# pabloruizponce/MixerMDM

Hardware: AMD Instinct MI355X
Metric: generated motions/sec (1000-step DDPM schedule sampled with DDIM eta=0, T=300, 2-person) (higher is better)
Workload: dtype f32; 1 GPU; BASELINE configs[2]: 2-person MixerMDM (in2IN individual + in2IN interaction + Mixer mode 4, align, CFG 3.5), T=300, ddim1000 (eta=0), batch 16 per GPU, fp32, random-init weights; batch_per_gpu=16, frames=300, sampler=ddim1000, sampler_steps=1000, hipgraph=True, parallelism=batch-sharded x1, no in-loop collective

## Files before the change

### include/mmdm.h

```cpp
#ifndef MMDM_H
#define MMDM_H

#include <stddef.h>
#include <stdint.h>

#ifdef __cplusplus
extern "C" {
#endif
#pragma GCC visibility push(default)

typedef enum {
    MMDM_OK = 0,
    MMDM_ERR_ARG = 1,
    MMDM_ERR_STATE = 2,
    MMDM_ERR_HIP = 3,
    MMDM_ERR_UNSUPPORTED = 4
} mmdm_status;

const char* mmdm_last_error(void);
const char* mmdm_version(void);
const char* mmdm_last_gemm_kernel(void);


enum {
// ... 205 lines not shown
    int noise_steps;
    const float* noise;
    const unsigned long long* item_seed;
    const int* item_noise_row;
    const float* x_start;
    const float* init_image;
    int init_zeros;
    float init_coef[2];
    int skip_timesteps;
} mmdm_begin_ragged_options;
int mmdm_begin_ragged_opts(mmdm_handle h, const float* cond, const float* x_T, int B, const int* lens_host, const mmdm_begin_ragged_options* opts, void* stream);
int mmdm_call_rows(mmdm_handle h, int* rows, int* real_rows, int* ragged);

int mmdm_set_history(mmdm_handle h, float* influence_i1, float* influence_i2, float* out1, float* out2, float* out_influenced, int every);

int mmdm_run(mmdm_handle h, int nsteps, int use_graph, void* stream);
int mmdm_graph_stats(mmdm_handle h, int64_t* captures, int64_t* replays, int* cached);
int mmdm_graph_parked(void);

int mmdm_seek(mmdm_handle h, int step_index, void* stream);

int mmdm_get_state(mmdm_handle h, float** x, float** x2, float** pred_xstart, float** pred_xstart2, float** model_out);

int mmdm_copy_result(mmdm_handle h, float* dst, void* stream);

int mmdm_module_forward(mmdm_handle h, int which, const float* x, const float* x2, const float* cond, int t,
                        float* out, int n, int T, void* stream);

int mmdm_profile_enable(mmdm_handle h, int on);
int mmdm_profile_read(mmdm_handle h, int which, double* total_ms, int64_t* launches, double* flops, double* algorithmic_bytes);

int mmdm_diag_set(const char* key, long long value);

#pragma GCC visibility pop
#ifdef __cplusplus
}
#endif
#endif
```

### mixermdm_amd/_lib.py

```python
import ctypes as C
import os

_HERE = os.path.dirname(os.path.abspath(__file__))
_LIB = None


class MMDMError(RuntimeError):

    def __init__(self, msg, status=0):
        super().__init__(msg)
        self.status = int(status)


def lib_path():
    return os.environ.get("MMDM_LIB") or os.path.join(_HERE, "libmmdm_hip.so")


def lib_override():
    return bool(os.environ.get("MMDM_LIB"))


class Config(C.Structure):
    _fields_ = [(n, C.c_int) for n in ("d_latent", "d_ff", "d_layers", "d_heads", "m_latent", "m_ff", "m_layers", "m_heads",
                                        "nfeats", "text_dim", "mixing_mode", "align", "xstart_align", "model2_kind", "use_force")] + \
# ... 71 lines not shown
    "mmdm_set_weight": (_I, [_VP, C.c_char_p, _VP, C.c_int64, C.c_int64, _VP]),
    "mmdm_set_norm_stats": (_I, [_VP, _VP]),
    "mmdm_set_schedule": (_I, [_VP, _VP, _VP, _I, _VP]),
    "mmdm_prepare": (_I, [_VP]),
    "mmdm_begin": (_I, [_VP, _VP, _VP, _I, _I, _VP]),
    "mmdm_set_eta": (_I, [_VP, _VP, _I]),
    "mmdm_begin_opts": (_I, [_VP, _VP, _VP, _I, _I, C.POINTER(BeginOptions), _VP]),
    "mmdm_randn_f32": (_I, [C.c_ulonglong, _I, _I, _I, _VP, _VP]),
    "mmdm_begin_ragged": (_I, [_VP, _VP, _VP, _I, _VP, _VP]),
    "mmdm_begin_ragged_opts": (_I, [_VP, _VP, _VP, _I, _VP, C.POINTER(BeginRaggedOptions), _VP]),
    "mmdm_call_rows": (_I, [_VP, C.POINTER(_I), C.POINTER(_I), C.POINTER(_I)]),
    "mmdm_attention_ragged_f32": (_I, [_VP, _I, _VP, _I, _VP, _I, _VP, _I, _I, _VP, _VP, _I, _I, _I, _I, _I, _VP]),
    "mmdm_attention_ragged_opts_f32": (_I, [_VP, _I, _VP, _I, _VP, _I, _VP, _I, _I, _I, _VP, _VP, _I, _I, _I, _I, _I, _VP]),
    "mmdm_attention_split_ragged": (_I, [_VP, _I, C.c_int64, _VP, _I, C.c_int64, _VP, _I, C.c_int64, _VP, _I, _I, _I, _I, _VP, _VP, _I, _I, _I, _I, _I, _VP]),
    "mmdm_layernorm_split": (_I, [_VP, _VP, _VP, _VP, _VP, C.c_int64, _I, _I, C.c_float, _I, _VP]),
    "mmdm_rowop_adaln": (_I, [_VP, _VP, _I, _I, _VP, _I, _VP, _I, _I, _I, _VP, _I, _I, _VP]),
    "mmdm_rowop_cond_silu": (_I, [_VP, _VP, _VP, _VP, _I, C.c_int64, _I, _I, _I, _VP]),
    "mmdm_rowop_mean_time": (_I, [_VP, _VP, _I, _I, _VP, _VP, _I, _I, _VP]),
    "mmdm_rowop_mdm_pack": (_I, [_VP, _VP, _I, _VP, _VP, _VP, _VP, _VP, C.c_int64, _I, _I, _I, _I, _VP]),
    "mmdm_rowop_mdm_unpack": (_I, [_VP, _VP, _I, _I, _I, _I, _VP]),
    "mmdm_rowop_mdm_pack_rag": (_I, [_VP, _VP, _I, _VP, _VP, _VP, _VP, _VP, C.c_int64, _I, _I, _I, _I] + [_I, _VP, _VP, _VP, _VP] * 2 + [_I, _VP]),
    "mmdm_rowop_mdm_unpack_rag": (_I, [_VP, _VP, _I, _I, _I] + [_I, _VP, _VP, _VP, _VP] * 2 + [_I, _VP]),
    "mmdm_set_history":(_I, [_VP, _VP, _VP, _VP, _VP, _VP, _I]),
    "mmdm_run": (_I, [_VP, _I, _I, _VP]),
    "mmdm_seek": (_I, [_VP, _I, _VP]),
    "mmdm_graph_stats": (_I, [_VP, C.POINTER(C.c_int64), C.POINTER(C.c_int64), C.POINTER(_I)]),
    "mmdm_graph_parked": (_I, []),
    "mmdm_last_gemm_kernel": (C.c_char_p, []),
    "mmdm_get_state": (_I, [_VP] + [C.POINTER(_VP)] * 5),
    "mmdm_copy_result": (_I, [_VP, _VP, _VP]),
    "mmdm_module_forward": (_I, [_VP, _I, _VP, _VP, _VP, _I, _VP, _I, _I, _VP]),
    "mmdm_profile_enable": (_I, [_VP, _I]),
    "mmdm_diag_set": (_I, [C.c_char_p, C.c_longlong]),
    "mmdm_profile_read": (_I, [_VP, _I, C.POINTER(C.c_double), C.POINTER(C.c_int64), C.POINTER(C.c_double), C.POINTER(C.c_double)]),
}


def load_library():
    global _LIB
    if _LIB is not None:
        return _LIB
    import torch
    path = lib_path()
    if not os.path.exists(path):
        raise MMDMError(f"{path} not found: build it with `python -m mixermdm_amd.build` (hipcc, gfx950). "
                        "There is no CPU fallback for the denoising path.")
    lib = C.CDLL(path)
    for name, (res, args) in SYMBOLS.items():
        fn = getattr(lib, name)
        fn.restype = res
        fn.argtypes = args
    _LIB = lib
    return lib


def diag(key, value):
    check(load_library().mmdm_diag_set(key.encode(), int(value)))


def check(rc, handle=None):
    if rc == 0:
        return
    lib = load_library()
    msg = (lib.mmdm_handle_error(handle) if handle else None) or lib.mmdm_last_error() or b""
    msg = msg.decode(errors="replace")
    if "Mixing mode not recognized" in msg or "Mode not recognized" in msg:
# ... 3 lines not shown
```

### mixermdm_amd/csrc/gemm_f32.hip

```cpp
#include <hip/hip_runtime.h>
#include <stdlib.h>
#include <string.h>
#include <type_traits>
#include "kernels.h"

namespace {

typedef float f32x16 __attribute__((ext_vector_type(16)));
typedef float f32x4 __attribute__((ext_vector_type(4)));
typedef unsigned u32x4 __attribute__((ext_vector_type(4)));

struct GemmArgs {
    const float* A; const float* W; const float* bias; float* C; const float* extra;
    int lda, ldw, ldc, ld_extra;
    int M, N, K, Kw, epilogue, period;
    int mt, nt;
    int ablate;
    unsigned long long* stamps;
};

template <int VEC, bool FULL>
__device__ __forceinline__ f32x4 load4(const float* __restrict__ base, int ld, int row, int nrows, int k, int K) {
    if (FULL) return *reinterpret_cast<const f32x4*>(base + (size_t)row * ld + k);
    f32x4 v = {0.f, 0.f, 0.f, 0.f};
// ... 145 lines not shown
                else if (p.epilogue == MMDM_EPI_BIAS_QUICKGELU) v = quick_gelu(v);
                else if (p.epilogue == MMDM_EPI_BIAS_SIGMOID) v = sigmoidf(v);
                p.C[(size_t)row * p.ldc + col] = v;
            }
        }
    }
}

template <int TM_, int TN_, int BK_ = 16, int NBUF_ = 2>
struct GCfg {
    static constexpr int WGM = TM_ / 10, WGN = TN_ / 10, TM = TM_ % 10, TN = TN_ % 10;
    static constexpr int NWAVES = WGM * WGN, THREADS = 64 * NWAVES;
    static constexpr int BM = 32 * TM * WGM, BN = 32 * TN * WGN, BK = BK_;
    static constexpr int A_FLOATS = BM * BK, B_FLOATS = BN * BK;
    static constexpr int NBUF = NBUF_;
    static constexpr int SMEM_BYTES = NBUF * (A_FLOATS + B_FLOATS) * 4;
    static constexpr int CPR = BK / 4;
    static constexpr int RPP = 64 / CPR;
    static constexpr int NA = BM / RPP, NB = BN / RPP;
    static constexpr int NI = (NA + NB) / NWAVES;
    static_assert((NA + NB) % NWAVES == 0, "pieces must divide evenly over the waves (counted vmcnt)");
    static constexpr int G = BK / 8;
};

typedef __attribute__((address_space(1))) const void* gptr_t;
typedef __attribute__((address_space(3))) void* lptr_t;

template <int CPR> __device__ __forceinline__ int swz_of(int r) { return CPR == 4 ? ((r >> 2) & 3) : ((r >> 1) & 7); }

template <int N> __device__ __forceinline__ void wait_vm() { asm volatile("s_waitcnt vmcnt(%0)" ::"n"(N) : "memory"); }

#if defined(__HIP_DEVICE_COMPILE__)
template <int TM_, int TN_, int BK_, int NBUF_, bool VEPI, int PIPE_, bool DIAG_>
__device__ __forceinline__ void gemm_tile(const GemmArgs& pp, float* smem, int swz, int bid) {
    using C_ = GCfg<TM_, TN_, BK_, NBUF_>;
    const GemmArgs& p = pp;
    unsigned long long* const p_stamps = DIAG_ ? pp.stamps : nullptr;
    const int p_ablate = DIAG_ ? pp.ablate : 0;
    constexpr int BM = C_::BM, BN = C_::BN, BK = C_::BK, TM = C_::TM, TN = C_::TN, CPR = C_::CPR, RPP = C_::RPP, NBUF = C_::NBUF;
    float* As = smem;
    float* Bs = smem + NBUF * C_::A_FLOATS;

    const int m0 = (swz / p.nt) * BM;
    const int n0 = (swz % p.nt) * BN;

    const int tid = threadIdx.x;
    const int lane = tid & 63;
    const int wave = __builtin_amdgcn_readfirstlane(tid >> 6);
    const int wm = wave / C_::WGN, wn = wave % C_::WGN;
    const int l31 = lane & 31, lh = lane >> 5;
    if (p_stamps && tid == 0) {
        p_stamps[8 * (size_t)bid + 0] = __builtin_amdgcn_s_memrealtime();
        p_stamps[8 * (size_t)bid + 3] = (unsigned long long)__builtin_amdgcn_s_getreg((4) | (0 << 6) | (31 << 11)) |
                                        ((unsigned long long)__builtin_amdgcn_s_getreg((20) | (0 << 6) | (3 << 11)) << 32);
    }

    constexpr int UA = C_::NA / C_::NWAVES;
    static_assert(C_::NA % C_::NWAVES == 0, "A pieces must divide evenly over the waves (compile-time operand of a piece)");
    int voff[C_::NI];
    int dst[C_::NI];
#pragma unroll
    for (int u = 0; u < C_::NI; ++u) {
        const int pq = wave + C_::NWAVES * u;
        const int prow = lane / CPR, pc = lane % CPR;
        const bool isa = u < UA;
        const int trow = (isa ? RPP * pq : RPP * (pq - C_::NA)) + prow;
        const int gch = pc ^ swz_of<CPR>(trow);
        if (isa) {
            const int rel = min(trow, p.M - 1 - m0);
            voff[u] = (rel * p.lda + 4 * gch) * 4;
            dst[u] = RPP * pq * BK;
        } else {
            const int rel = min(trow, p.N - 1 - n0);
            voff[u] = (rel * p.ldw + 4 * gch) * 4;
            dst[u] = NBUF * C_::A_FLOATS + RPP * (pq - C_::NA) * BK;
        }
    }
    const __amdgpu_buffer_rsrc_t rsA = __builtin_amdgcn_make_buffer_rsrc(const_cast<float*>(p.A + (size_t)m0 * p.lda), 0, 0xffffffff, 0x00020000);
    const __amdgpu_buffer_rsrc_t rsW = __builtin_amdgcn_make_buffer_rsrc(const_cast<float*>(p.W + (size_t)n0 * p.ldw), 0, 0xffffffff, 0x00020000);
    int koff = 0;
    auto stage_part = [&](int buf, auto u0c, auto u1c) {
        constexpr int u0 = decltype(u0c)::value, u1 = decltype(u1c)::value;
#pragma unroll
        for (int u = u0; u < u1; ++u) {
            const int boff = u < UA ? buf * C_::A_FLOATS : buf * C_::B_FLOATS;
            __builtin_amdgcn_raw_ptr_buffer_load_lds(u < UA ? rsA : rsW, (lptr_t)(smem + dst[u] + boff), 16, voff[u], koff, 0, 0);
        }
        if constexpr (u1 == C_::NI) koff += BK * 4;
    };
    auto stage = [&](int buf) { stage_part(buf, std::integral_constant<int, 0>{}, std::integral_constant<int, C_::NI>{}); };

    const int nkt = p.K / BK;
    constexpr bool LATE_R = PIPE_ != 0 && VEPI;
    f32x16 acc[TM][TN];
    if (VEPI) {
#pragma unroll
        for (int i = 0; i < TM; ++i) {
            const int row = m0 + wm * (32 * TM) + i * 32 + l31;
            const bool rok = row < p.M;
            const int er = p.epilogue == MMDM_EPI_BIAS_PE ? row % p.period : row;
            const bool ext = !LATE_R && (p.epilogue == MMDM_EPI_BIAS_RESID || p.epilogue == MMDM_EPI_BIAS_PE) && rok;
#pragma unroll
            for (int j = 0; j < TN; ++j)
#pragma unroll
                for (int qd = 0; qd < 4; ++qd) {
                    const int col = n0 + wn * (32 * TN) + j * 32 + 8 * qd + 4 * lh;
                    f32x4 v = {0.f, 0.f, 0.f, 0.f};
                    if (col < p.N) {
                        if (p.bias) v = *reinterpret_cast<const f32x4*>(p.bias + col);
                        if (ext) v += *reinterpret_cast<const f32x4*>(p.extra + (size_t)er * p.ld_extra + col);
                    }
#pragma unroll
                    for (int c = 0; c < 4; ++c) acc[i][j][4 * qd + c] = v[c];
                }
        }
    } else {
#pragma unroll
    for (int i = 0; i < TM; ++i)
#pragma unroll
        for (int j = 0; j < TN; ++j) {
            const int col = n0 + wn * (32 * TN) + j * 32 + l31;
            const bool cok = col < p.N;
            const float bv = (p.bias && cok) ? p.bias[col] : 0.f;
#pragma unroll
            for (int e = 0; e < 16; ++e) {
                float v = bv;
                if (p.epilogue == MMDM_EPI_BIAS_RESID || p.epilogue == MMDM_EPI_BIAS_PE) {
                    const int row = m0 + wm * (32 * TM) + i * 32 + (e & 3) + 8 * (e >> 2) + 4 * lh;
                    if (cok && row < p.M) {
                        const int er = p.epilogue == MMDM_EPI_BIAS_PE ? row % p.period : row;
                        v += p.extra[(size_t)er * p.ld_extra + col];
                    }
                }
                acc[i][j][e] = v;
            }
        }
    }

    if constexpr (PIPE_ != 0) {
#pragma unroll
        for (int t = 0; t < NBUF - 1; ++t) stage(t);
        wait_vm<(NBUF - 2) * C_::NI>();
    } else {
        asm volatile("s_waitcnt vmcnt(0)" ::: "memory");
    }
    if (p_stamps && tid == 0) {
        p_stamps[8 * (size_t)bid + 1] = __builtin_amdgcn_s_memrealtime();
        p_stamps[8 * (size_t)gridDim.x + 2 * bid] = __builtin_readcyclecounter();
    }
    const int sw = swz_of<CPR>(l31);
    const int a_row = (wm * (32 * TM) + l31) * BK;
    const int b_row = (wn * (32 * TN) + l31) * BK;

    f32x4 rv[LATE_R ? TM : 1][LATE_R ? TN : 1][4];
    if constexpr (PIPE_ != 0) {
        static_assert((C_::G == 2 || C_::G == 4) && NBUF >= 3 && NBUF <= 6, "pipelined loop: K step 16 or 32 (two / four k-groups), 3 to 6 stages");
        static_assert((C_::NI + 1) / 2 <= 4 * TM * TN - 1, "LDS-DMA pieces of a tile must fit behind the MFMAs of two k-groups");
        constexpr int NI = C_::NI;
        f32x4 a0[TM], b0[TN], a1[TM], b1[TN];
        auto rd = [&](int buf, int g, f32x4 (&af)[TM], f32x4 (&bf)[TN]) {
            const int cg = 4 * ((2 * g + lh) ^ sw);
            const float* Ac = As + buf * C_::A_FLOATS + a_row + cg;
            const float* Bc = Bs + buf * C_::B_FLOATS + b_row + cg;
// ... 49 lines not shown
            } else {
                if constexpr (g < G - 1) rd(cur, g + 1, a0, b0);
                else if (more) rd(nxt, 0, a0, b0);
                if constexpr (STG && g == 1 && PIPE_ != 2) stage_part(stg, std::integral_constant<int, D0>{}, std::integral_constant<int, NI>{});
                mm(a1, b1);
            }
            __builtin_amdgcn_sched_group_barrier(0x008, 1, g);
            __builtin_amdgcn_sched_group_barrier(0x100, TM + TN, g);
#pragma unroll
            for (int u = 0; u < dma_here; ++u) {
                __builtin_amdgcn_sched_group_barrier(0x008, 1, g);
                __builtin_amdgcn_sched_group_barrier(0x010, 1, g);
            }
            __builtin_amdgcn_sched_group_barrier(0x008, NMM - 1 - dma_here, g);
            __builtin_amdgcn_sched_barrier(0);
        };
        auto step = [&](auto do_stage, int left, bool more) {
            group(std::integral_constant<int, 0>{}, do_stage, left, more);
            group(std::integral_constant<int, 1>{}, do_stage, left, more);
            if constexpr (G >= 4) {
                group(std::integral_constant<int, 2>{}, do_stage, left, more);
                group(std::integral_constant<int, 3>{}, do_stage, left, more);
            }
            cur = nxt; nxt = nxt + 1 == NBUF ? 0 : nxt + 1;
        };
        for (int kt = 0; kt < n_main; ++kt) {
            step(std::true_type{}, 0, true);
            stg = stg + 1 == NBUF ? 0 : stg + 1;
        }
        if constexpr (LATE_R) {
#pragma unroll
            for (int i = 0; i < TM; ++i) {
                const int row = m0 + wm * (32 * TM) + i * 32 + l31;
                const int er = p.epilogue == MMDM_EPI_BIAS_PE ? row % p.period : row;
#pragma unroll
                for (int j = 0; j < TN; ++j)
#pragma unroll
                    for (int qd = 0; qd < 4; ++qd) {
                        const int col = n0 + wn * (32 * TN) + j * 32 + 8 * qd + 4 * lh;
                        const int rr = row < p.M ? er : 0, cc = col < p.N ? col : 0;
                        rv[i][j][qd] = *reinterpret_cast<const f32x4*>(p.extra + (size_t)rr * p.ld_extra + cc);
                    }
            }
        }
        for (int kt = n_main < 0 ? 0 : n_main; kt < nkt; ++kt)
            step(std::false_type{}, nkt - kt - 2, kt + 1 < nkt);
    } else {
    stage(0);
    if (NBUF == 3 && nkt > 1) stage(1);
    for (int kt = 0; kt < nkt; ++kt) {
        const int cur = NBUF == 3 ? kt % 3 : (kt & 1);
        if (NBUF == 3) {
            if (kt + 1 < nkt) asm volatile("s_waitcnt vmcnt(%0)" ::"n"(C_::NI) : "memory");
            else asm volatile("s_waitcnt vmcnt(0)" ::: "memory");
            asm volatile("s_waitcnt lgkmcnt(0)" ::: "memory");
            __builtin_amdgcn_s_barrier();
            if (kt + 2 < nkt && (p_ablate & 7) < 1) stage((kt + 2) % 3);
        } else {
            asm volatile("s_waitcnt vmcnt(0)" ::: "memory");
            __syncthreads();
            if (kt + 1 < nkt && (p_ablate & 7) < 1) stage(cur ^ 1);
        }
        const float* Ac = As + ((p_ablate & 7) >= 1 ? 0 : cur) * C_::A_FLOATS + a_row;
        const float* Bc = Bs + ((p_ablate & 7) >= 1 ? 0 : cur) * C_::B_FLOATS + b_row;
#pragma unroll
        for (int g = 0; g < C_::G; ++g) {
            const int cg = 4 * ((2 * g + lh) ^ sw);
// ... 353 lines not shown
template <int TM_, int TN_, int BK_ = 16, int NBUF_ = 2, int MINW_ = 1, int PIPE_ = 0>
int launch_glds(GemmArgs a, hipStream_t st) {
    using C_ = GCfg<TM_, TN_, BK_, NBUF_>;
    a.mt = (a.M + C_::BM - 1) / C_::BM;
    a.nt = (a.N + C_::BN - 1) / C_::BN;
    const bool ext = a.epilogue == MMDM_EPI_BIAS_RESID || a.epilogue == MMDM_EPI_BIAS_PE;
    const bool vepi = ext && vepi_ok(a) && !(a.ablate & 16);
    const dim3 grid(a.mt * a.nt), block(C_::THREADS);
    mmdm_note_gemm("%s<%d,%d,%d,%d,%s>", PIPE_ ? "gemm_pipe" : "gemm_glds", TM_, TN_, BK_, NBUF_, vepi ? "vepi" : "scalar");
    if ((a.ablate & ~16) || a.stamps) {
        if (vepi) hipLaunchKernelGGL((gemm_glds_kernel<TM_, TN_, BK_, NBUF_, true, MINW_, PIPE_, true>), grid, block, C_::SMEM_BYTES, st, a);
        else hipLaunchKernelGGL((gemm_glds_kernel<TM_, TN_, BK_, NBUF_, false, MINW_, PIPE_, true>), grid, block, C_::SMEM_BYTES, st, a);
    } else if (vepi)
        hipLaunchKernelGGL((gemm_glds_kernel<TM_, TN_, BK_, NBUF_, true, MINW_, PIPE_, false>), grid, block, C_::SMEM_BYTES, st, a);
    else
        hipLaunchKernelGGL((gemm_glds_kernel<TM_, TN_, BK_, NBUF_, false, MINW_, PIPE_, false>), grid, block, C_::SMEM_BYTES, st, a);
    return mmdm_check_launch("gemm_glds");
}

template <int TM_, int TN_, int BK_ = 16, int NBUF_ = 2, int MINW_ = 1, int PIPE_ = 0>
int set_attr_glds() {
    constexpr int bytes = GCfg<TM_, TN_, BK_, NBUF_>::SMEM_BYTES;
    const void* fns[4] = {reinterpret_cast<const void*>(&gemm_glds_kernel<TM_, TN_, BK_, NBUF_, true, MINW_, PIPE_, false>),
                          reinterpret_cast<const void*>(&gemm_glds_kernel<TM_, TN_, BK_, NBUF_, false, MINW_, PIPE_, false>),
                          reinterpret_cast<const void*>(&gemm_glds_kernel<TM_, TN_, BK_, NBUF_, true, MINW_, PIPE_, true>),
                          reinterpret_cast<const void*>(&gemm_glds_kernel<TM_, TN_, BK_, NBUF_, false, MINW_, PIPE_, true>)};
    for (const void* f : fns) {
        hipError_t e = hipFuncSetAttribute(f, hipFuncAttributeMaxDynamicSharedMemorySize, bytes);
        if (e != hipSuccess) return mmdm_set_error(MMDM_ERR_HIP, "hipFuncSetAttribute(gemm_glds): %s", hipGetErrorString(e));
    }
    return MMDM_OK;
}

template <int TM, int TN, int BK, int AVEC, int WVEC, bool FULL>
int set_attr() {
    hipError_t e = hipFuncSetAttribute(reinterpret_cast<const void*>(&gemm_f32_kernel<TM, TN, BK, AVEC, WVEC, FULL>),
                                       hipFuncAttributeMaxDynamicSharedMemorySize, Cfg<TM, TN, BK>::SMEM_BYTES);
    if (e != hipSuccess) return mmdm_set_error(MMDM_ERR_HIP, "hipFuncSetAttribute(gemm): %s", hipGetErrorString(e));
    return MMDM_OK;
}

template <int TM, int TN, int BK, int AVEC, int WVEC, bool FULL>
int launch(GemmArgs a, hipStream_t st) {
    using C_ = Cfg<TM, TN, BK>;
    a.mt = (a.M + C_::BM - 1) / C_::BM;
    a.nt = (a.N + C_::BN - 1) / C_::BN;
    mmdm_note_gemm("gemm_f32<%d,%d,%d>", TM, TN, BK);
    hipLaunchKernelGGL((gemm_f32_kernel<TM, TN, BK, AVEC, WVEC, FULL>), dim3(a.mt * a.nt), dim3(C_::THREADS), C_::SMEM_BYTES, st, a);
    return mmdm_check_launch("gemm_f32");
}

template <int TM, int TN, int BK>
int launch_cfg(const GemmArgs& a, bool av, bool wv, hipStream_t st) {
    using C_ = Cfg<TM, TN, BK>;
    const bool full = av && wv && (a.M % C_::BM == 0) && (a.N % C_::BN == 0) && (a.K % C_::BK == 0) && a.Kw == a.K;
    if (full) return launch<TM, TN, BK, 4, 4, true>(a, st);
    if (av && wv) return launch<TM, TN, BK, 4, 4, false>(a, st);
    if (!av && wv) return launch<TM, TN, BK, 1, 4, false>(a, st);
    if (av && !wv) return launch<TM, TN, BK, 4, 1, false>(a, st);
    return launch<TM, TN, BK, 1, 1, false>(a, st);
}

template <int TM, int TN, int BK>
int set_attr_cfg() {
    int rc;
    if ((rc = set_attr<TM, TN, BK, 4, 4, true>())) return rc;
    if ((rc = set_attr<TM, TN, BK, 4, 4, false>())) return rc;
    if ((rc = set_attr<TM, TN, BK, 1, 4, false>())) return rc;
    if ((rc = set_attr<TM, TN, BK, 4, 1, false>())) return rc;
    return set_attr<TM, TN, BK, 1, 1, false>();
}

inline bool vec_ok(const float* p, int ld, int K) {
    return (reinterpret_cast<uintptr_t>(p) & 15) == 0 && (ld & 3) == 0 && (K & 3) == 0;
}

}

int g_gemm_cfg = -1;
int g_gemm_tail = -1;
static thread_local int t_gemm_tail = 0;
void mmdm_gemm_set_tail(int t) { t_gemm_tail = t; }
int mmdm_gemm_get_tail(void) { return t_gemm_tail; }
int g_gemm_ablate = 0;
#ifndef MMDM_S16_DEFAULT
#define MMDM_S16_DEFAULT -1
#endif
int g_gemm_s16 = MMDM_S16_DEFAULT;
unsigned long long* g_gemm_stamps = nullptr;

int mmdm_gemm_init(void) {
    int rc;
    if ((rc = set_attr_cfg<22, 22, 32>())) return rc;
    if ((rc = set_attr_cfg<22, 22, 16>())) return rc;
    if ((rc = set_attr_cfg<22, 12, 16>())) return rc;
    if ((rc = set_attr_cfg<22, 22, 8>())) return rc;
    if ((rc = set_attr_cfg<42, 22, 16>())) return rc;
    if ((rc = set_attr_cfg<22, 42, 16>())) return rc;
    if ((rc = set_attr_glds<42, 22>())) return rc;
    if ((rc = set_attr_glds<22, 22>())) return rc;
    if ((rc = set_attr_glds<22, 21>())) return rc;
    if ((rc = set_attr_glds<22, 22, 16, 4, 1, 1>())) return rc;
    if ((rc = set_attr_glds<42, 22, 16, 3, 1, 1>())) return rc;
    if ((rc = set_attr_glds<22, 21, 16, 3, 1, 1>())) return rc;
    if ((rc = set_attr_glds<22, 22, 16, 5, 1, 1>())) return rc;
    if ((rc = set_attr_glds<22, 21, 16, 4, 1, 1>())) return rc;
    if ((rc = set_attr_glds<22, 21, 16, 5, 1, 1>())) return rc;
    if ((rc = set_attr_glds<21, 21, 16, 4, 1, 1>())) return rc;
    if ((rc = set_attr_glds<22, 22, 16, 5, 1, 2>())) return rc;
    if ((rc = set_attr_glds<22, 22, 16, 5, 1, 3>())) return rc;
    if ((rc = set_attr_s16<1, 3>())) return rc;
    if ((rc = set_attr_s16<2, 3>())) return rc;
    if ((rc = set_attr_s16<1, 4>())) return rc;
    if ((rc = set_attr_s16<2, 4>())) return rc;
    if ((rc = set_attr_mix())) return rc;
    return MMDM_OK;
}

bool mmdm_diag_gemm_f32(const char* key, long long v) {
    if (!strcmp(key, "gemm_cfg")) g_gemm_cfg = (int)v;
    else if (!strcmp(key, "gemm_ablate")) g_gemm_ablate = (int)v;
    else if (!strcmp(key, "gemm_tail")) g_gemm_tail = (int)v;
    else if (!strcmp(key, "gemm_s16")) g_gemm_s16 = (int)v;
    else if (!strcmp(key, "gemm_stamps")) g_gemm_stamps = reinterpret_cast<unsigned long long*>((uintptr_t)v);
    else return false;
    return true;
}

extern "C" int mmdm_linear_f32(const float* A, int lda, const float* W, int ldw, const float* bias, float* C, int ldc,
                               int M, int N, int K, int epilogue, const float* extra, int ld_extra, int period, void* stream) {
    return mmdm_linear_f32_ex(A, lda, W, ldw, K, bias, C, ldc, M, N, K, epilogue, extra, ld_extra, period, stream);
}

int mmdm_linear_f32_ex(const float* A, int lda, const float* W, int ldw, int Kw, const float* bias, float* C, int ldc,
                       int M, int N, int K, int epilogue, const float* extra, int ld_extra, int period, void* stream) {
    mmdm_note_gemm_reset();
    if (M == 0 || N == 0) return MMDM_OK;
    if (int rc = mmdm_kernels_init()) return rc;
    if (!A || !W || !C || M < 0 || N < 0 || K <= 0 || lda < K || ldw < Kw || Kw < K || ldc < N)
        return mmdm_set_error(MMDM_ERR_ARG, "mmdm_linear_f32: bad shape M=%d N=%d K=%d lda=%d ldw=%d ldc=%d", M, N, K, lda, ldw, ldc);
    if (epilogue < MMDM_EPI_BIAS || epilogue > MMDM_EPI_BIAS_SIGMOID)
        return mmdm_set_error(MMDM_ERR_ARG, "mmdm_linear_f32: unknown epilogue %d", epilogue);
    if ((epilogue == MMDM_EPI_BIAS_RESID || epilogue == MMDM_EPI_BIAS_PE) && (!extra || ld_extra < N))
        return mmdm_set_error(MMDM_ERR_ARG, "mmdm_linear_f32: epilogue %d needs `extra` with ld >= N", epilogue);
    if (epilogue == MMDM_EPI_BIAS_PE && period <= 0)
        return mmdm_set_error(MMDM_ERR_ARG, "mmdm_linear_f32: PE epilogue needs period > 0");
    GemmArgs a;
    a.A = A; a.W = W; a.bias = bias; a.C = C; a.extra = extra;
    a.lda = lda; a.ldw = ldw; a.ldc = ldc; a.ld_extra = ld_extra;
    a.M = M; a.N = N; a.K = K; a.Kw = Kw; a.epilogue = epilogue; a.period = period > 0 ? period : 1;
    a.mt = a.nt = 0;
    a.ablate = g_gemm_ablate;
    a.stamps = g_gemm_stamps;
    hipStream_t st = static_cast<hipStream_t>(stream);
    const bool av = vec_ok(A, lda, K), wv = vec_ok(W, ldw, Kw);
    const bool glds_ok = av && wv && (K % 16 == 0) && Kw == K;
    const int tail = g_gemm_tail >= 0 ? g_gemm_tail : t_gemm_tail;
    switch (g_gemm_cfg) {
        case 10: if (glds_ok) return launch_glds<42, 22>(a, st); break;
        case -1:
            if (glds_ok && K >= 96 && tail && epilogue != MMDM_EPI_BIAS_PE) {
                const bool narrow = N <= 512 || K <= 512 || N == 2048;
                const long slots = narrow ? 768 : 512, nt = (N + (narrow ? 63 : 127)) / (narrow ? 64 : 128), mt = (M + 127) / 128;
                const long tiles = mt * nt, full = tiles / slots, rem = tiles - full * slots;
                const long mt1 = full * slots / nt;
                if ((long)((M + 127) / 128) * ((N + 63) / 64) >= 512 && full >= 1 && mt1 >= 1 && mt1 < mt && rem * 10 <= slots * tail) {
                    const int M1 = (int)mt1 * 128;
                    GemmArgs b = a;
                    a.M = M1;
                    b.M = M - M1;
                    b.A = A + (size_t)M1 * lda;
                    b.C = C + (size_t)M1 * ldc;
                    if (extra) b.extra = extra + (size_t)M1 * ld_extra;
                    int rc = narrow ? launch_glds<22, 21, 16, 4, 1, 1>(a, st) : launch_glds<22, 22, 16, 5, 1, 1>(a, st);
                    if (rc) return rc;
                    const long r128 = (long)((b.M + 127) / 128) * ((N + 63) / 64);
                    if (!narrow && r128 >= 256) return launch_glds<22, 21, 16, 4, 1, 1>(b, st);
                    return launch_glds<21, 21, 16, 4, 1, 1>(b, st);
                }
            }
            if (glds_ok && K >= 96) {
                const long t64 = (long)((M + 127) / 128) * ((N + 63) / 64);
                if (g_gemm_s16 > 0 && s16_ok(a)) {
                    switch (g_gemm_s16) {
                        case 13: return launch_s16<1, 3>(a, st);
                        case 14: return launch_s16<1, 4>(a, st);
                        case 24: return launch_s16<2, 4>(a, st);
                        default: return launch_s16<2, 3>(a, st);
                    }
                }
                if (g_gemm_s16 < 0 && (long)((M + 63) / 64) * ((N + 63) / 64) <= 128 && !(M <= 64 && N >= 4096) && s16_ok(a)) return launch_s16<1, 4>(a, st);
                if (t64 < 512 && g_gemm_s16 < 0 && epilogue != MMDM_EPI_BIAS_PE && s16_ok(a) && vepi_ok(a)) {
                    const long nt64 = (N + 63) / 64, tiles = (long)((M + 63) / 64) * nt64, rounds = tiles / 256, mt1 = rounds * 256 / nt64;
// ... 37 lines not shown
```

### mixermdm_amd/csrc/kernels.h

```cpp
#pragma once
#include <hip/hip_runtime.h>
#include <stdint.h>
#include "../../include/mmdm.h"

int mmdm_set_error(int code, const char* fmt, ...) __attribute__((format(printf, 2, 3)));
int mmdm_check_launch(const char* what);
int mmdm_kernels_init(void);
void mmdm_note_gemm(const char* fmt, ...) __attribute__((format(printf, 1, 2)));
void mmdm_note_gemm_reset(void);
int mmdm_gemm_init(void);
void mmdm_gemm_set_tail(int t);
int mmdm_gemm_get_tail(void);
int mmdm_gemm_bf16_init(void);
int mmdm_gemm_split_init(void);
bool mmdm_diag_gemm_f32(const char* key, long long v);
bool mmdm_diag_gemm_bf16(const char* key, long long v);
bool mmdm_diag_gemm_split(const char* key, long long v);
bool mmdm_diag_attn(const char* key, long long v);

__device__ __forceinline__ float erf_bf(float a) {
    const float t = __builtin_fabsf(a), s = a * a;
    float r = __builtin_fmaf(-1.72853470e-5f, t, 3.83197126e-4f);
    const float u = __builtin_fmaf(-3.88396438e-3f, t, 2.42546219e-2f);
    r = __builtin_fmaf(r, s, u);
    r = __builtin_fmaf(r, t, -1.06777877e-1f);
    r = __builtin_fmaf(r, t, -6.34846687e-1f);
    r = __builtin_fmaf(r, t, -1.28717512e-1f);
    r = __builtin_fmaf(r, t, -t);
    r = 1.0f - __builtin_amdgcn_exp2f(r * 1.44269504088896340736f);
    r = __builtin_copysignf(r, a);
    float q = -5.96761703e-4f;
    q = __builtin_fmaf(q, s, 4.99119423e-3f);
    q = __builtin_fmaf(q, s, -2.67681349e-2f);
    q = __builtin_fmaf(q, s, 1.12819925e-1f);
    q = __builtin_fmaf(q, s, -3.76125336e-1f);
    q = __builtin_fmaf(q, s, 1.28379166e-1f);
    q = __builtin_fmaf(q, a, a);
    return t > 0.927734375f ? r : q;
}
__device__ __forceinline__ float gelu_erf(float x) {
    const float h = 0.5f * x;
    return __builtin_fmaf(h, erf_bf(x * 0.70710678118654752440f), h);
}
__device__ __forceinline__ float sigmoidf(float x) { return 1.0f / (1.0f + expf(-x)); }
__device__ __forceinline__ float silu(float x) { return x / (1.0f + expf(-x)); }
// ... 120 lines not shown
```

### mixermdm_amd/csrc/mmdm.hip

```cpp
#include <hip/hip_runtime.h>
#include <stdarg.h>
#include <stdio.h>
#include <stdlib.h>
#include <string.h>
#include <atomic>
#include <memory>
#include <mutex>
#include <shared_mutex>
#include <string>
#include <unordered_map>
#include <vector>
#include "kernels.h"

static thread_local char g_err[512] = "";

int mmdm_set_error(int code, const char* fmt, ...) {
    va_list ap;
    va_start(ap, fmt);
    vsnprintf(g_err, sizeof(g_err), fmt, ap);
    va_end(ap);
    return code;
}

int mmdm_check_launch(const char* what) {
// ... 408 lines not shown
            RC(dalloc(h, &q, (size_t)F * D)); e.l1_s = q;
            RC(dalloc(h, &q, (size_t)D * F)); e.l2_s = q;
        }
        const std::string b = pfx + "seqTransEncoder.layers." + std::to_string(i) + ".";
        RC(add_slot(h, b + "self_attn.in_proj_weight", &e.in_w, 3 * D, D));
        RC(add_slot(h, b + "self_attn.in_proj_bias", &e.in_b, 3 * D, 1));
        RC(add_slot(h, b + "self_attn.out_proj.weight", &e.out_w, D, D));
        RC(add_slot(h, b + "self_attn.out_proj.bias", &e.out_b, D, 1));
        RC(add_slot(h, b + "linear1.weight", &e.l1_w, F, D));
        RC(add_slot(h, b + "linear1.bias", &e.l1_b, F, 1));
        RC(add_slot(h, b + "linear2.weight", &e.l2_w, D, F));
        RC(add_slot(h, b + "linear2.bias", &e.l2_b, D, 1));
        RC(add_slot(h, b + "norm1.weight", &e.n1_g, D, 1));
        RC(add_slot(h, b + "norm1.bias", &e.n1_b, D, 1));
        RC(add_slot(h, b + "norm2.weight", &e.n2_g, D, 1));
        RC(add_slot(h, b + "norm2.bias", &e.n2_b, D, 1));
    }
    return MMDM_OK;
}

struct Ctx {
    mmdm_handle h;
    hipStream_t st;
    const Scratch* s;
    const Geom* g = nullptr;
    const unsigned char* kmask = nullptr;
    const int* klast = nullptr;
    int kmask_rows = 0;
    bool rag() const { return g && g->rag; }
    size_t rows_of(int nseq, int T) const { return g ? g->rows_of(nseq) : (size_t)nseq * T; }
};

struct TailScope {
    int prev;
    explicit TailScope(int t) : prev(mmdm_gemm_get_tail()) { mmdm_gemm_set_tail(t); }
    ~TailScope() { mmdm_gemm_set_tail(prev); }
};

int prof_begin(const Ctx& c, int cls, double flops, double bytes = 0) {
    if (!c.h) return MMDM_OK;
    Prof& p = c.h->prof;
    if (!p.on) return MMDM_OK;
    if (p.used[cls] + 2 > p.ev[cls].size()) {
        for (int i = 0; i < 2; ++i) {
            hipEvent_t e;
            HIPCHK(hipEventCreate(&e));
            p.ev[cls].push_back(e);
        }
    }
    p.flops[cls] += flops;
    p.bytes[cls] += bytes;
    HIPCHK(hipEventRecord(p.ev[cls][p.used[cls]], c.st));
    return MMDM_OK;
}

int prof_end(const Ctx& c, int cls) {
    if (!c.h) return MMDM_OK;
    Prof& p = c.h->prof;
    if (!p.on) return MMDM_OK;
    HIPCHK(hipEventRecord(p.ev[cls][p.used[cls] + 1], c.st));
    p.used[cls] += 2;
    return MMDM_OK;
}

int linear(const Ctx& c, const float* A, int lda, const float* W, int ldw, const float* bias, float* C, int ldc, int M, int N, int K,
           int epi = MMDM_EPI_BIAS, const float* extra = nullptr, int ld_extra = 0, int period = 0, int Kw = 0) {
    const int cls = c.h && c.h->cfg.precision != 0 ? 3 : 0;
    RC(prof_begin(c, cls, 2.0 * M * N * K, 4.0 * ((double)M * K + (double)N * K + (double)M * N * (epi == MMDM_EPI_BIAS_RESID ? 2 : 1))));
    RC(mmdm_linear_f32_ex(A, lda, W, ldw, Kw ? Kw : K, bias, C, ldc, M, N, K, epi, extra, ld_extra, period, c.st));
    return prof_end(c, cls);
// ... 346 lines not shown
        StackRun r1 = r, r2 = r;
        r1.nseq = r2.nseq = n;
        r1.sa_rows = r2.sa_rows = n;
        r2.sa_row0 = n;
        r2.kv_src = H->mI + nT * Dm;
        HIPCHK(hipEventRecord(H->ev_fork2, c.st));
        HIPCHK(hipStreamWaitEvent(H->st2, H->ev_fork2, 0));
        RC(run_stack(c2, H->mx.st, c.s->h + nT * Dm, r2));
        RC(run_stack(c, H->mx.st, c.s->h, r1));
        HIPCHK(hipEventRecord(H->ev_join2, H->st2));
        HIPCHK(hipStreamWaitEvent(c.st, H->ev_join2, 0));
    } else {
        RC(run_stack(c, H->mx.st, c.s->h, r));
    }
    const int mode = cf.mixing_mode;
    if (mode == 1 || mode == 3) {
        if (rag) RC(ROWOP(c, mmdm_mean_time_rag, c.s->h, H->hpool, 2 * n, c.g->seq_off, c.g->seq_len, Dm, c.st));
        else RC(ROWOP(c, mmdm_mean_time_f32, c.s->h, H->hpool, 2 * n, T, Dm, c.st));
        RC(linear(c, H->hpool, Dm, H->mx.out_w, Dm, H->mx.out_b, H->w23, H->nw, 2 * n, H->nw, Dm, MMDM_EPI_BIAS_SIGMOID));
    } else {
        RC(linear(c, c.s->h, Dm, H->mx.out_w, Dm, H->mx.out_b, H->w23, H->nw, (int)(2 * nT), H->nw, Dm, MMDM_EPI_BIAS_SIGMOID));
    }
    const int* lp = H->d_step + 1;
    if (rag) RC(mmdm_blend_cfg_rag(H->out1, H->out2, H->w23, mode, cf.use_force, cf.force_val, cf.cfg_scale, H->model_out, H->d_hist, lp, c.g->rg, c.st));
    else RC(mmdm_blend_cfg_dyn(H->out1, H->out2, H->w23, mode, cf.use_force, cf.force_val, cf.cfg_scale, H->model_out, H->d_hist, lp, B, T, c.st));
    RC(mmdm_hist_copy(H->out1, H->d_hist, 0, nT * NF2, lp, c.st));
    RC(mmdm_hist_copy(H->out2, H->d_hist, 1, nT * NF2, lp, c.st));
    return MMDM_OK;
}

int run_step(const Ctx& c) {
    mmdm_handle H = c.h;
    const int B = H->B, T = H->T, n = 2 * B;
    TailScope tail_scope((H->cfg.single_only == 1 || H->cfg.single_only == 2) ? 10 : 0);
    if (H->cfg.single_only == 1) {
        if (H->d1.kind == 1) {
            RC(run_denoiser_mdm(c, H->d1, H->x, B, 1, NF, n, T, H->cond_cat, H->td1, H->o1, NF));
        } else {
            RC(cond_vectors(c, H->d1, H->txt_d1, H->se_d1, H->ss_d1, n));
            RC(run_denoiser(c, H->d1, false, H->x, B, 1, NF, n, T, H->ss_d1, ss_ld_of(H->d1), H->o1, NF));
        }
        if (c.rag()) RC(mmdm_cfg_ddim_f32(H->o1, H->d_coef, H->S, H->d_step, H->cfg.cfg_scale, H->x, H->px1, 1, c.g->rows, NF, c.st));
        else RC(mmdm_cfg_ddim_f32(H->o1, H->d_coef, H->S, H->d_step, H->cfg.cfg_scale, H->x, H->px1, B, T, NF, c.st));
        return mmdm_step_dec(H->d_step, H->d_step + 1, c.st);
    }
    if (H->cfg.single_only == 2) {
        const int n4 = 4 * B;
        RC(cond_vectors(c, H->d2, H->txt_d2, H->se_d2, H->ss_d2, 3 * n4));
        RC(run_denoiser(c, H->d2, true, H->x, B, 2, NF2, n4, T, H->ss_d2, ss_ld_of(H->d2), H->o2, NF2));
        RC(mmdm_cfg4_ddim_f32(H->o2, H->d_coef, H->S, H->d_step, H->cfg.cfg_scale, H->cfg.cfg_scale_interaction, H->cfg.cfg_scale_individual,
                              H->x, H->px1, B, T, NF2, c.st));
        return mmdm_step_dec(H->d_step, H->d_step + 1, c.st);
    }
    const bool dual = H->cfg.single_only == 3;
    if (H->pinned) RC(c.rag() ? mmdm_pin_root_rag(H->x, H->x2, H->d_opts, c.g->rg, c.st) : mmdm_pin_root(H->x, H->x2, H->d_opts, B, T, c.st));
    auto model1 = [&](const Ctx& cc) -> int {
        if (H->d1.kind == 1) return run_denoiser_mdm(cc, H->d1, H->x, B, 2, NF2, n, T, H->cond_cat + 3 * H->cfg.text_dim, H->cond_w, H->o1, NF2);
        if (dual) return run_dual_individual(cc, H->d1, H->x, B, n, T, H->ss_d1, ss_ld_of(H->d1), H->o1);
        return run_denoiser(cc, H->d1, false, H->x, B, 2, NF2, n, T, H->ss_d1, ss_ld_of(H->d1), H->o1, NF2);
    };
    const float* xin2 = dual ? H->x : H->x2;
    if (H->overlap && !H->prof.on) {
        Ctx c2{H, H->st2, &H->sb, c.g, c.kmask, c.klast, c.kmask_rows};
        HIPCHK(hipEventRecord(H->ev_fork, c.st));
        HIPCHK(hipStreamWaitEvent(H->st2, H->ev_fork, 0));
        RC(cond_vectors(c2, H->d2, H->txt_d2, H->se_d2, H->ss_d2, 3 * n));
        RC(run_denoiser(c2, H->d2, true, xin2, B, 2, NF2, n, T, H->ss_d2, ss_ld_of(H->d2), H->o2, NF2));
// ... 781 lines not shown
    return MMDM_OK;
}

extern "C" int mmdm_copy_result(mmdm_handle h, float* dst, void* stream) {
    if (!h || !dst) return mmdm_set_error(MMDM_ERR_ARG, "mmdm_copy_result: null argument");
    if (!h->begun) return herr(h, mmdm_set_error(MMDM_ERR_STATE, "mmdm_copy_result: call mmdm_begin / mmdm_begin_ragged first"));
    const float* src = h->cfg.single_only ? h->px1 : h->px2;
    const size_t n = (size_t)h->geom.real_rows * (h->cfg.single_only == 1 ? NF : NF2);
    HIPCHK(hipMemcpyAsync(dst, src, n * sizeof(float), hipMemcpyDeviceToDevice, static_cast<hipStream_t>(stream)));
    return MMDM_OK;
}

extern "C" int mmdm_module_forward(mmdm_handle h, int which, const float* x, const float* x2, const float* cond, int t,
                                   float* out, int n, int T, void* stream) {
    if (!h || !x || !cond || !out) return mmdm_set_error(MMDM_ERR_ARG, "mmdm_module_forward: null argument");
    if (!h->prepared) return herr(h, mmdm_set_error(MMDM_ERR_STATE, "mmdm_module_forward: call mmdm_prepare first"));
    const int so_ = h->cfg.single_only;
    const bool cfgx2 = which == 4;
    if (cfgx2) {
        if (so_ != 0) return herr(h, mmdm_set_error(MMDM_ERR_ARG, "mmdm_module_forward: module 4 (CFG x2) needs the two-chain handle"));
        if (n <= 0 || n > h->cfg.max_batch || T <= 0 || T > h->cfg.max_frames)
            return herr(h, mmdm_set_error(MMDM_ERR_ARG, "mmdm_module_forward: B=%d (<= max_batch) T=%d out of range", n, T));
    } else if (n <= 0 || (n & 1) || n / 2 > h->cfg.max_batch * (so_ == 2 ? 2 : 1) || T <= 0 || T > h->cfg.max_frames)
        return herr(h, mmdm_set_error(MMDM_ERR_ARG, "mmdm_module_forward: n=%d (even, <= 2*max_batch) T=%d out of range", n, T));
    if (t < 0 || t >= 5000) return herr(h, mmdm_set_error(MMDM_ERR_ARG, "mmdm_module_forward: timestep %d out of range", t));
    if (which < 0 || which > 4 || (so_ == 1 && which != 0) || (so_ == 2 && which != 1) || (so_ == 3 && (which == 2 || which == 0)) || (so_ != 3 && which == 3)) return herr(h, mmdm_set_error(MMDM_ERR_ARG, "mmdm_module_forward: bad module %d", which));
    hipStream_t st = static_cast<hipStream_t>(stream);
    Ctx c{h, st, &h->sa};
    if (h->mask_rows && which == 3) return herr(h, mmdm_set_error(MMDM_ERR_UNSUPPORTED, "mmdm_module_forward: module 3 (dual_individual) takes no key mask"));
    RC(herr(h, use_key_mask(h, c, n, T, "mmdm_module_forward")));
    h->call_stream = st;
    const int td = h->cfg.text_dim;
    ProfPause pause(h->prof);
    TailScope tail_scope((so_ == 1 || so_ == 2) ? 10 : 0);
    const int S_keep = h->S;
    ModuleW* mods[3] = {so_ != 2 ? &h->d1 : nullptr, so_ != 1 ? &h->d2 : nullptr, so_ == 0 ? &h->mx : nullptr};
    const size_t Dst = max2(max2(h->d1.st.D, h->d2.st.D), h->mx.st.D);
    if (S_keep > 0)
        for (int k = 0; k < 3; ++k)
            if (mods[k]) HIPCHK(hipMemcpyAsync(h->tt_stash + k * Dst, mods[k]->time_tab, mods[k]->st.D * sizeof(float), hipMemcpyDeviceToDevice, st));
    int rc = MMDM_OK;
    auto done = [&](int code) {
        h->S = S_keep;
        if (S_keep > 0) {
            hipError_t e = hipMemcpyAsync(h->d_tmap, &h->h_tmap0, sizeof(int), hipMemcpyHostToDevice, st);
            for (int k = 0; k < 3 && e == hipSuccess; ++k)
                if (mods[k]) e = hipMemcpyAsync(mods[k]->time_tab, h->tt_stash + k * Dst, mods[k]->st.D * sizeof(float), hipMemcpyDeviceToDevice, st);
            if (e == hipSuccess) e = hipStreamSynchronize(st);
            if (e != hipSuccess && !code) code = mmdm_set_error(MMDM_ERR_HIP, "mmdm_module_forward: restoring the schedule tables failed: %s", hipGetErrorString(e));
        }
        return herr(h, code);
    };
    h->S = 1;
    h->begun = false;
    {
        hipError_t e = hipMemcpyAsync(h->d_tmap, &t, sizeof(int), hipMemcpyHostToDevice, st);
        if (e == hipSuccess) e = hipStreamSynchronize(st);
        if (e != hipSuccess) return done(mmdm_set_error(MMDM_ERR_HIP, "mmdm_module_forward: timestep upload failed: %s", hipGetErrorString(e)));
        if ((rc = mmdm_set_step(h->d_step, h->d_step + 1, 0, 0, st))) return done(rc);
    }
    if (which == 3) {
        if ((rc = build_time_tab(c, h->d1))) return done(rc);
        if ((rc = text_rows(c, h->d1, cond, 5 * td, 3 * td, h->txt_d1, 0, n))) return done(rc);
        if ((rc = text_rows(c, h->d1, cond, 5 * td, 4 * td, h->txt_d1, n, n))) return done(rc);
        if ((rc = cond_vectors(c, h->d1, h->txt_d1, h->se_d1, h->ss_d1, 2 * n))) return done(rc);
        rc = run_dual_individual(c, h->d1, x, n, n, T, h->ss_d1, ss_ld_of(h->d1), out);
        return done(rc);
// ... 158 lines not shown
```

Before: 0.2681 motions/s.

## Add mixed-tile GEMM launch that runs the last partial wave with smaller tiles

Adds a fused GEMM kernel whose grid holds full-size tiles for the first M1 rows and smaller 64-row tiles for the remainder, chosen by a planner so that the large-tile part fills an exact number of CU waves and the remainder spreads over more workgroups. The aim is to cut the wave-quantization tail where a small fraction of large tiles leaves most CUs idle in the last wave. The positional-encoding epilogue gets a row offset so the remainder rows index the period table correctly. It is on by default for the two-chain path (mode 1) and the single paths (11), and it adds planner heuristics plus risk of slower small tiles when the thresholds are wrong.

Result: no change. 0.2707 motions/s (median of 6 runs) (+1.0%).

```diff
diff --git a/include/mmdm.h b/include/mmdm.h
--- a/include/mmdm.h
+++ b/include/mmdm.h
@@ -261,6 +261,8 @@
 
 int mmdm_diag_set(const char* key, long long value);
 
+int mmdm_gemm_mixtail_plan(int M, int N, int K, int tile, int cus, int wgs_per_cu, int max_frac_pct, int* M1, int* rem_tile);
+
 #pragma GCC visibility pop
 #ifdef __cplusplus
 }
diff --git a/mixermdm_amd/_lib.py b/mixermdm_amd/_lib.py
--- a/mixermdm_amd/_lib.py
+++ b/mixermdm_amd/_lib.py
@@ -127,6 +127,7 @@
     "mmdm_module_forward": (_I, [_VP, _I, _VP, _VP, _VP, _I, _VP, _I, _I, _VP]),
     "mmdm_profile_enable": (_I, [_VP, _I]),
     "mmdm_diag_set": (_I, [C.c_char_p, C.c_longlong]),
+    "mmdm_gemm_mixtail_plan": (_I, [_I, _I, _I, _I, _I, _I, _I, C.POINTER(_I), C.POINTER(_I)]),
     "mmdm_profile_read": (_I, [_VP, _I, C.POINTER(C.c_double), C.POINTER(C.c_int64), C.POINTER(C.c_double), C.POINTER(C.c_double)]),
 }
 
diff --git a/mixermdm_amd/csrc/gemm_f32.hip b/mixermdm_amd/csrc/gemm_f32.hip
--- a/mixermdm_amd/csrc/gemm_f32.hip
+++ b/mixermdm_amd/csrc/gemm_f32.hip
@@ -201,7 +201,7 @@
 
 #if defined(__HIP_DEVICE_COMPILE__)
 template <int TM_, int TN_, int BK_, int NBUF_, bool VEPI, int PIPE_, bool DIAG_>
-__device__ __forceinline__ void gemm_tile(const GemmArgs& pp, float* smem, int swz, int bid) {
+__device__ __forceinline__ void gemm_tile(const GemmArgs& pp, float* smem, int swz, int bid, int row0 = 0) {
     using C_ = GCfg<TM_, TN_, BK_, NBUF_>;
     const GemmArgs& p = pp;
     unsigned long long* const p_stamps = DIAG_ ? pp.stamps : nullptr;
@@ -267,7 +267,7 @@
         for (int i = 0; i < TM; ++i) {
             const int row = m0 + wm * (32 * TM) + i * 32 + l31;
             const bool rok = row < p.M;
-            const int er = p.epilogue == MMDM_EPI_BIAS_PE ? row % p.period : row;
+            const int er = p.epilogue == MMDM_EPI_BIAS_PE ? (row + row0) % p.period : row;
             const bool ext = !LATE_R && (p.epilogue == MMDM_EPI_BIAS_RESID || p.epilogue == MMDM_EPI_BIAS_PE) && rok;
 #pragma unroll
             for (int j = 0; j < TN; ++j)
@@ -297,7 +297,7 @@
                 if (p.epilogue == MMDM_EPI_BIAS_RESID || p.epilogue == MMDM_EPI_BIAS_PE) {
                     const int row = m0 + wm * (32 * TM) + i * 32 + (e & 3) + 8 * (e >> 2) + 4 * lh;
                     if (cok && row < p.M) {
-                        const int er = p.epilogue == MMDM_EPI_BIAS_PE ? row % p.period : row;
+                        const int er = p.epilogue == MMDM_EPI_BIAS_PE ? (row + row0) % p.period : row;
                         v += p.extra[(size_t)er * p.ld_extra + col];
                     }
                 }
@@ -413,7 +413,7 @@
 #pragma unroll
             for (int i = 0; i < TM; ++i) {
                 const int row = m0 + wm * (32 * TM) + i * 32 + l31;
-                const int er = p.epilogue == MMDM_EPI_BIAS_PE ? row % p.period : row;
+                const int er = p.epilogue == MMDM_EPI_BIAS_PE ? (row + row0) % p.period : row;
 #pragma unroll
                 for (int j = 0; j < TN; ++j)
 #pragma unroll
@@ -833,6 +833,54 @@
     return MMDM_OK;
 }
 
+struct MixTailArgs { GemmArgs main, rem; int n_main, row0; };
+
+template <int TN_, int NBUF_, bool VEPI>
+__global__ __launch_bounds__(256) void gemm_mixtail_kernel(MixTailArgs q) {
+#if defined(__HIP_DEVICE_COMPILE__)
+    extern __shared__ __attribute__((aligned(16))) float smem[];
+    const int bid = blockIdx.x;
+    if (bid < q.n_main) gemm_tile<22, TN_, 16, NBUF_, VEPI, 1, false>(q.main, smem, xcd_swz(bid, q.n_main), bid);
+    else gemm_tile<21, 21, 16, 4, VEPI, 1, false>(q.rem, smem, xcd_swz(bid - q.n_main, q.rem.mt * q.rem.nt), bid, q.row0);
+#endif
+}
+
+template <int TN_, int NBUF_>
+int launch_mixtail(const GemmArgs& a, int M1, hipStream_t st) {
+    using CM = GCfg<22, TN_, 16, NBUF_>;
+    using CR = GCfg<21, 21, 16, 4>;
+    static_assert(CM::SMEM_BYTES >= CR::SMEM_BYTES && CM::THREADS == CR::THREADS, "the remainder form runs inside the main form's launch configuration");
+    MixTailArgs q;
+    q.main = a; q.rem = a;
+    q.main.M = M1;
+    q.rem.M = a.M - M1;
+    q.rem.A = a.A + (size_t)M1 * a.lda;
+    q.rem.C = a.C + (size_t)M1 * a.ldc;
+    if (a.extra && a.epilogue == MMDM_EPI_BIAS_RESID) q.rem.extra = a.extra + (size_t)M1 * a.ld_extra;
+    q.row0 = a.epilogue == MMDM_EPI_BIAS_PE ? M1 % a.period : 0;
+    q.main.mt = (M1 + CM::BM - 1) / CM::BM; q.main.nt = (a.N + CM::BN - 1) / CM::BN;
+    q.rem.mt = (q.rem.M + CR::BM - 1) / CR::BM; q.rem.nt = (a.N + CR::BN - 1) / CR::BN;
+    q.main.ablate = q.rem.ablate = 0; q.main.stamps = q.rem.stamps = nullptr;
+    q.n_main = q.main.mt * q.main.nt;
+    const bool ext = a.epilogue == MMDM_EPI_BIAS_RESID || a.epilogue == MMDM_EPI_BIAS_PE;
+    const bool vepi = ext && vepi_ok(a);
+    mmdm_note_gemm("gemm_mixtail<22,%d,16,%d|21,21,16,4,%s,%d+%d>", TN_, NBUF_, vepi ? "vepi" : "scalar", q.n_main, q.rem.mt * q.rem.nt);
+    const dim3 grid(q.n_main + q.rem.mt * q.rem.nt), block(CM::THREADS);
+    if (vepi) hipLaunchKernelGGL((gemm_mixtail_kernel<TN_, NBUF_, true>), grid, block, CM::SMEM_BYTES, st, q);
+    else hipLaunchKernelGGL((gemm_mixtail_kernel<TN_, NBUF_, false>), grid, block, CM::SMEM_BYTES, st, q);
+    return mmdm_check_launch("gemm_mixtail");
+}
+
+template <int TN_, int NBUF_>
+int set_attr_mixtail() {
+    const void* fns[2] = {reinterpret_cast<const void*>(&gemm_mixtail_kernel<TN_, NBUF_, true>), reinterpret_cast<const void*>(&gemm_mixtail_kernel<TN_, NBUF_, false>)};
+    for (const void* f : fns) {
+        hipError_t e = hipFuncSetAttribute(f, hipFuncAttributeMaxDynamicSharedMemorySize, GCfg<22, TN_, 16, NBUF_>::SMEM_BYTES);
+        if (e != hipSuccess) return mmdm_set_error(MMDM_ERR_HIP, "hipFuncSetAttribute(gemm_mixtail): %s", hipGetErrorString(e));
+    }
+    return MMDM_OK;
+}
+
 template <int TM, int TN, int BK, int AVEC, int WVEC, bool FULL>
 int set_attr() {
     hipError_t e = hipFuncSetAttribute(reinterpret_cast<const void*>(&gemm_f32_kernel<TM, TN, BK, AVEC, WVEC, FULL>),
@@ -878,11 +926,20 @@
 
 }
 
+static constexpr int kCUs = 256;
 int g_gemm_cfg = -1;
 int g_gemm_tail = -1;
 static thread_local int t_gemm_tail = 0;
 void mmdm_gemm_set_tail(int t) { t_gemm_tail = t; }
 int mmdm_gemm_get_tail(void) { return t_gemm_tail; }
+#ifndef MMDM_MIXTAIL_DEFAULT
+#define MMDM_MIXTAIL_DEFAULT -1
+#endif
+int g_gemm_mixtail = MMDM_MIXTAIL_DEFAULT;
+int g_gemm_mixtail_rows = 0;
+static thread_local int t_gemm_mixtail = 0;
+void mmdm_gemm_set_mixtail(int v) { t_gemm_mixtail = v; }
+int mmdm_gemm_get_mixtail(void) { return t_gemm_mixtail; }
 int g_gemm_ablate = 0;
 #ifndef MMDM_S16_DEFAULT
 #define MMDM_S16_DEFAULT -1
@@ -915,6 +972,27 @@
     if ((rc = set_attr_s16<1, 4>())) return rc;
     if ((rc = set_attr_s16<2, 4>())) return rc;
     if ((rc = set_attr_mix())) return rc;
+    if ((rc = set_attr_mixtail<22, 5>())) return rc;
+    if ((rc = set_attr_mixtail<21, 4>())) return rc;
+    return MMDM_OK;
+}
+
+extern "C" int mmdm_gemm_mixtail_plan(int M, int N, int K, int tile, int cus, int wgs_per_cu, int max_frac_pct, int* M1, int* rem_tile) {
+    if (!M1 || !rem_tile || (tile != 128 && tile != 64) || M < 0 || N <= 0 || K <= 0 || cus <= 0 || wgs_per_cu <= 0 || max_frac_pct < 0 || max_frac_pct > 100)
+        return mmdm_set_error(MMDM_ERR_ARG, "mmdm_gemm_mixtail_plan: bad argument (M=%d N=%d K=%d tile=%d cus=%d wgs_per_cu=%d max_frac_pct=%d)", M, N, K, tile, cus,
+                              wgs_per_cu, max_frac_pct);
+    *M1 = M;
+    *rem_tile = 0;
+    const long slots = (long)cus * wgs_per_cu, nt = (N + tile - 1) / tile, mt = (M + 127) / 128;
+    const long tiles = mt * nt, full = tiles / slots, frac = tiles - full * slots;
+    if (full < 1 || frac == 0) return MMDM_OK;
+    const long mt1 = full * slots / nt;
+    if (mt1 < 1 || mt1 >= mt) return MMDM_OK;
+    const long rem = (mt - mt1) * nt;
+    const long thr = max_frac_pct ? max_frac_pct : tile == 128 ? 50 : (K <= 512 && N >= 1024) ? 100 : 0;
+    if (rem * 100 > slots * thr) return MMDM_OK;
+    *M1 = (int)mt1 * 128;
+    *rem_tile = 64;
     return MMDM_OK;
 }
 
@@ -923,6 +1001,8 @@
     else if (!strcmp(key, "gemm_ablate")) g_gemm_ablate = (int)v;
     else if (!strcmp(key, "gemm_tail")) g_gemm_tail = (int)v;
     else if (!strcmp(key, "gemm_s16")) g_gemm_s16 = (int)v;
+    else if (!strcmp(key, "gemm_mixtail")) g_gemm_mixtail = (int)v;
+    else if (!strcmp(key, "gemm_mixtail_rows")) g_gemm_mixtail_rows = (int)v;
     else if (!strcmp(key, "gemm_stamps")) g_gemm_stamps = reinterpret_cast<unsigned long long*>((uintptr_t)v);
     else return false;
     return true;
@@ -957,9 +1037,21 @@
     const bool av = vec_ok(A, lda, K), wv = vec_ok(W, ldw, Kw);
     const bool glds_ok = av && wv && (K % 16 == 0) && Kw == K;
     const int tail = g_gemm_tail >= 0 ? g_gemm_tail : t_gemm_tail;
+    const int mixt = g_gemm_mixtail >= 0 ? g_gemm_mixtail : t_gemm_mixtail;
     switch (g_gemm_cfg) {
         case 10: if (glds_ok) return launch_glds<42, 22>(a, st); break;
         case -1:
+            if (glds_ok && K >= 96 && mixt > 0 && !a.ablate && !a.stamps) {
+                const int sel = mixt % 10;
+                const bool narrow = sel == 3 || (sel != 2 && (N <= 512 || K <= 512 || N == 2048));
+                int M1 = 0, rt = 0;
+                if (g_gemm_mixtail_rows > 0) {
+                    if (g_gemm_mixtail_rows % 128 == 0 && g_gemm_mixtail_rows < M) { M1 = g_gemm_mixtail_rows; rt = 64; }
+                } else if ((long)((M + 127) / 128) * ((N + 63) / 64) >= 512 && !(M <= 256 && N >= 4096)) {
+                    if (int rc = mmdm_gemm_mixtail_plan(M, N, K, narrow ? 64 : 128, kCUs, narrow ? 3 : 2, mixt >= 10 ? 100 : 0, &M1, &rt)) return rc;
+                }
+                if (rt && M1 > 0 && M1 < M) return narrow ? launch_mixtail<21, 4>(a, M1, st) : launch_mixtail<22, 5>(a, M1, st);
+            }
             if (glds_ok && K >= 96 && tail && epilogue != MMDM_EPI_BIAS_PE) {
                 const bool narrow = N <= 512 || K <= 512 || N == 2048;
                 const long slots = narrow ? 768 : 512, nt = (N + (narrow ? 63 : 127)) / (narrow ? 64 : 128), mt = (M + 127) / 128;
diff --git a/mixermdm_amd/csrc/kernels.h b/mixermdm_amd/csrc/kernels.h
--- a/mixermdm_amd/csrc/kernels.h
+++ b/mixermdm_amd/csrc/kernels.h
@@ -11,6 +11,8 @@
 int mmdm_gemm_init(void);
 void mmdm_gemm_set_tail(int t);
 int mmdm_gemm_get_tail(void);
+void mmdm_gemm_set_mixtail(int v);
+int mmdm_gemm_get_mixtail(void);
 int mmdm_gemm_bf16_init(void);
 int mmdm_gemm_split_init(void);
 bool mmdm_diag_gemm_f32(const char* key, long long v);
diff --git a/mixermdm_amd/csrc/mmdm.hip b/mixermdm_amd/csrc/mmdm.hip
--- a/mixermdm_amd/csrc/mmdm.hip
+++ b/mixermdm_amd/csrc/mmdm.hip
@@ -464,10 +464,16 @@
 };
 
 struct TailScope {
-    int prev;
-    explicit TailScope(int t) : prev(mmdm_gemm_get_tail()) { mmdm_gemm_set_tail(t); }
-    ~TailScope() { mmdm_gemm_set_tail(prev); }
+    int prev, prev_mix;
+    TailScope(int t, int mix) : prev(mmdm_gemm_get_tail()), prev_mix(mmdm_gemm_get_mixtail()) { mmdm_gemm_set_tail(t); mmdm_gemm_set_mixtail(mix); }
+    ~TailScope() { mmdm_gemm_set_tail(prev); mmdm_gemm_set_mixtail(prev_mix); }
 };
+#ifndef MMDM_MIXTAIL_SINGLE
+#define MMDM_MIXTAIL_SINGLE 11
+#endif
+#ifndef MMDM_MIXTAIL_DUAL
+#define MMDM_MIXTAIL_DUAL 1
+#endif
 
 int prof_begin(const Ctx& c, int cls, double flops, double bytes = 0) {
     if (!c.h) return MMDM_OK;
@@ -880,7 +886,8 @@
 int run_step(const Ctx& c) {
     mmdm_handle H = c.h;
     const int B = H->B, T = H->T, n = 2 * B;
-    TailScope tail_scope((H->cfg.single_only == 1 || H->cfg.single_only == 2) ? 10 : 0);
+    const bool one_stream = H->cfg.single_only == 1 || H->cfg.single_only == 2;
+    TailScope tail_scope(one_stream ? 10 : 0, one_stream ? MMDM_MIXTAIL_SINGLE : MMDM_MIXTAIL_DUAL);
     if (H->cfg.single_only == 1) {
         if (H->d1.kind == 1) {
             RC(run_denoiser_mdm(c, H->d1, H->x, B, 1, NF, n, T, H->cond_cat, H->td1, H->o1, NF));
@@ -1728,7 +1735,7 @@
     h->call_stream = st;
     const int td = h->cfg.text_dim;
     ProfPause pause(h->prof);
-    TailScope tail_scope((so_ == 1 || so_ == 2) ? 10 : 0);
+    TailScope tail_scope((so_ == 1 || so_ == 2) ? 10 : 0, (so_ == 1 || so_ == 2) ? MMDM_MIXTAIL_SINGLE : MMDM_MIXTAIL_DUAL);
     const int S_keep = h->S;
     ModuleW* mods[3] = {so_ != 2 ? &h->d1 : nullptr, so_ != 1 ? &h->d2 : nullptr, so_ == 0 ? &h->mx : nullptr};
     const size_t Dst = max2(max2(h->d1.st.D, h->d2.st.D), h->mx.st.D);
```
